# ChaoqinRobotics/LINS---LiDAR-inertial-SLAM

Hardware: AMD Instinct MI355X
Metric: ESKF iterations/sec (16x1800 VLP-16, ~2k feat) (higher is better)
Workload: dtype f64 state / f32 points

## Files before the change

### lins---lidar-inertial-slam_amd/csrc/debug_kernels.hip

```cpp
#include <hip/hip_runtime.h>

#include "ieskf_device.h"
#include "ieskf_rowsum.h"
#include "icp_wave.h"
#include "lins_launch.h"

namespace lins {

__global__ void debug_math_kernel(int op, int n, int n_in, int n_out, const double* __restrict__ in, double* __restrict__ out) {
  const int i = blockIdx.x * blockDim.x + threadIdx.x;
  if (i >= n) return;
  const double* a = in + (size_t)i * n_in;
  double* o = out + (size_t)i * n_out;
  if (op == 0) {
    const V3 v = quat2axis(Q4{a[0], a[1], a[2], a[3]});
    o[0] = v.x, o[1] = v.y, o[2] = v.z;
  } else if (op == 1) {
    const Q4 q = axis2quat(V3{a[0], a[1], a[2]});
    o[0] = q.w, o[1] = q.x, o[2] = q.y, o[3] = q.z;
  } else if (op == 2) {
    const M3 m = rinvleft(V3{a[0], a[1], a[2]});
    for (int k = 0; k < 9; ++k) o[k] = m.m[k];
  } else if (op == 3) {
    double s[19];
    for (int k = 0; k < 19; ++k) s[k] = a[k];
    box_plus_inplace(s, a + 19);
    for (int k = 0; k < 19; ++k) o[k] = s[k];
  } else if (op == 4) {
    IterConst ic;
    for (int k = 0; k < 19; ++k) ic.lin[k] = a[19 + k];
    make_iter_const(a, ic);
    for (int k = 0; k < 18; ++k) o[k] = ic.d[k];
  } else if (op == 5) {
    V3 phi;
    M3 gt;
    phi_and_Gt(Q4{a[0], a[1], a[2], a[3]}, phi, gt);
    o[0] = phi.x, o[1] = phi.y, o[2] = phi.z;
    for (int k = 0; k < 9; ++k) o[3 + k] = gt.m[k];
  } else if (op == 7) {
    double m[6][7], x6[6];
    for (int r = 0; r < 6; ++r)
      for (int c = 0; c < 7; ++c) m[r][c] = a[r * 7 + c];
    reg_solve6(m, x6);
    for (int k = 0; k < 6; ++k) o[k] = x6[k];
  } else if (op == 11) {
    double m[6][7], x6[6];
    for (int r = 0; r < 6; ++r)
      for (int c = 0; c < 7; ++c) m[r][c] = a[r * 7 + c];
    gj_solve6(m, x6);
    for (int k = 0; k < 6; ++k) o[k] = x6[k];
  } else if (op == 13) {
    const Q4 q = axis2quat_fast(V3{a[0], a[1], a[2]});
    o[0] = q.w, o[1] = q.x, o[2] = q.y, o[3] = q.z;
  } else if (op == 14) {
    const V3 v = quat2axis_fast(Q4{a[0], a[1], a[2], a[3]});
    o[0] = v.x, o[1] = v.y, o[2] = v.z;
  } else if (op == 15) {
    V3 phi;
    M3 gt;
    phi_and_Gt_general(Q4{a[0], a[1], a[2], a[3]}, phi, gt);
    o[0] = phi.x, o[1] = phi.y, o[2] = phi.z;
    for (int k = 0; k < 9; ++k) o[3 + k] = gt.m[k];
  } else if (op == 6) {
    DevParams prm{};
    prm.inv_period = (double)(1.f / (float)a[23]);
    const V3 phi = quat2axis(Q4{a[6], a[7], a[8], a[9]});
    float x, y, z;
    transform_to_start(prm, phi, V3{a[0], a[1], a[2]}, make_float4((float)a[19], (float)a[20], (float)a[21], (float)a[22]), x, y, z);
    o[0] = x, o[1] = y, o[2] = z;
  }
}

__global__ __launch_bounds__(256) void debug_cycles_kernel(int op, const double* __restrict__ in, double* __restrict__ out) {
  const int tid = threadIdx.x;
  DevParams prm{};
  prm.inv_period = 10.0, prm.icp_freq = 1, prm.lidar_scale = 1.0;
  V3 phi{in[0], in[1], in[2]}, t{in[3], in[4], in[5]};
  float4 q = make_float4((float)in[6] + tid * 0.01f, (float)in[7], (float)in[8], 3.05f);
  float acc = 0.f;
  double dacc = 0.0;
  const long long t0 = clock64();
#pragma unroll 1
  for (int r = 0; r < 64; ++r) {
    if (op == 100) {
      float x, y, z;
      transform_to_start(prm, phi, t, q, x, y, z);
      q.x = x * 0.999f + acc * 1e-9f, acc += y + z;
    } else if (op == 101) {
      QueryOut o;
      o.accepted = 0;
      o.c[0] = o.c[1] = o.c[2] = o.c[3] = 0.f;
      surf_row(prm, 1, q.x, q.y, q.z, make_float4(1.f + acc, 2.f, 3.f, 0.f), make_float4(1.5f, 2.2f, 3.f, 0.f), make_float4(1.f, 2.6f, 3.1f, 0.f), o);
      acc += o.c[0] * 1e-3f + o.c[3];
    } else if (op == 102) {
      double row[7] = {dacc + 1.0, 2.0, 3.0, 4.0, 5.0, 6.0, 7.0 + tid};
      dacc += wave_reduce_rows(row, tid & 63) * 1e-9;
    } else if (op == 103) {
      if ((tid & 63) == 0) {
        double a[6][7], x6[6];
        for (int i = 0; i < 6; ++i)
          for (int j = 0; j < 7; ++j) a[i][j] = (i == j ? 10.0 : 0.1 * (i + j)) + dacc;
        reg_solve6(a, x6);
        dacc += x6[0] * 1e-9;
      }
    } else if (op == 105) {
      const int l = tid & 63, i = l / 7, j = l % 7;
      double x6[6];
      wave_solve6(l < 42 ? (i == j ? 10.0 : 0.1 * (i + j)) + dacc : 0.0, l, x6);
      dacc += x6[0] * 1e-9;
    } else if (op == 106) {
      const int l = tid & 63, i = l / 7, j = l % 7;
      double x6[6];
      wave_gj_solve6(l < 42 ? (i == j ? 10.0 : 0.1 * (i + j)) + dacc : 0.0, l, x6);
      dacc += x6[0] * 1e-9;
    } else if (op == 107) {
      V3 p2;
      M3 gt;
      phi_and_Gt_general(Q4{1.0 - dacc, 0.01, 0.02, 0.03 + dacc}, p2, gt);
      dacc += (p2.x + gt.m[1]) * 1e-9;
    } else if (op == 108) {
      const Q4 r = axis2quat(V3{0.001 + dacc, 0.002, 0.003});
      dacc += (r.x + r.w) * 1e-9;
    } else if (op == 109) {
      const Q4 r = axis2quat_fast(V3{0.001 + dacc, 0.002, 0.003});
      dacc += (r.x + r.w) * 1e-9;
    } else if (op == 110) {
      const V3 r = quat2axis(Q4{1.0 - dacc, 0.001, 0.002, 0.003});
      dacc += r.x * 1e-9;
    } else if (op == 111) {
      const V3 r = quat2axis_fast(Q4{1.0 - dacc, 0.001, 0.002, 0.003});
      dacc += r.x * 1e-9;
    } else if (op == 104) {
      V3 p2;
      M3 gt;
      phi_and_Gt(Q4{1.0 - dacc, 0.01, 0.02, 0.03 + dacc}, p2, gt);
      dacc += (p2.x + gt.m[1]) * 1e-9;
    }
  }
  const long long t1 = clock64();
  if (tid == 0) out[blockIdx.x * 2] = (double)(t1 - t0) / 64.0, out[blockIdx.x * 2 + 1] = (double)acc + dacc;
}

__global__ void debug_wave_solve_kernel(int n, int gj, const double* __restrict__ in, double* __restrict__ out) {
  const int item = blockIdx.x, l = threadIdx.x;
  double x6[6];
  if (gj)
    wave_gj_solve6(l < 42 ? in[(size_t)item * 42 + l] : 0.0, l, x6);
  else
    wave_solve6(l < 42 ? in[(size_t)item * 42 + l] : 0.0, l, x6);
  if (l < 6) out[(size_t)item * 6 + l] = x6[l];
}
__device__ __forceinline__ double reduce_rows_ref(const double (&row)[7], int lane) {
  constexpr int A[28] = {0, 0, 0, 0, 0, 0, 1, 1, 1, 1, 1, 2, 2, 2, 2, 3, 3, 3, 4, 4, 5, 0, 1, 2, 3, 4, 5, 6};
  constexpr int B[28] = {0, 1, 2, 3, 4, 5, 1, 2, 3, 4, 5, 2, 3, 4, 5, 3, 4, 5, 4, 5, 5, 6, 6, 6, 6, 6, 6, 6};
  double v[28];
  for (int k = 0; k < 28; ++k) v[k] = row[A[k]] * row[B[k]];
  int cnt = 14;
  for (int m = 32; m >= 2; m >>= 1) {
    const bool up = (lane & m) != 0;
    if (m == 8) v[7] = 0.0;
    for (int i = 0; i < cnt; ++i) {
      const double lo = v[i], hi = v[i + cnt];
      v[i] = (up ? hi : lo) + shfl_xor_f64(up ? lo : hi, m);
    }
    cnt = m == 16 ? 4 : cnt / 2;
  }
  return v[0] + shfl_xor_f64(v[0], 1);
}
__global__ void debug_reduce_rows_kernel(int op, const double* __restrict__ in, double* __restrict__ out) {
  const int item = blockIdx.x, l = threadIdx.x;
  double row[7];
  for (int k = 0; k < 7; ++k) row[k] = in[((size_t)item * 64 + l) * 7 + k];
  const double acc = op == 9 ? wave_reduce_rows(row, l) : reduce_rows_ref(row, l);
  const int idx = reduce_sum_index(l);
  if (idx >= 0) out[(size_t)item * 28 + idx] = acc;
}
void launch_debug_reduce_rows(hipStream_t stream, int op, int n, const double* in, double* out) {
  hipLaunchKernelGGL(debug_reduce_rows_kernel, dim3(n), dim3(64), 0, stream, op, in, out);
}

__global__ void debug_icp_gn_kernel(int wave_version, const double* __restrict__ in, double* __restrict__ out) {
  __shared__ double ws[kIcpWorkspace + 48];
  const int item = blockIdx.x, l = threadIdx.x;
  const double* a = in + (size_t)item * 43;
  double* JTJ = ws + kIcpWorkspace;
  if (l < 42) JTJ[l] = a[l];
  __syncthreads();
  const int iter = (int)a[42];
  if (wave_version) {
    double x[6];
    wave_icp_gn_solve(JTJ, JTJ + 36, iter, l, x, ws);
    if (l == 0)
      for (int k = 0; k < 6; ++k) out[(size_t)item * 6 + k] = x[k];
  } else if (l == 0) {
    double* x = JTJ + 42;
    icp_gn_solve(JTJ, JTJ + 36, iter, x, ws);
    for (int k = 0; k < 6; ++k) out[(size_t)item * 6 + k] = x[k];
  }
}
void launch_debug_icp_gn(hipStream_t stream, int n, int wave_version, const double* in, double* out) {
  hipLaunchKernelGGL(debug_icp_gn_kernel, dim3(n), dim3(64), 0, stream, wave_version, in, out);
}

void launch_debug_wave_solve(hipStream_t stream, int n, int gj, const double* in, double* out) {
  hipLaunchKernelGGL(debug_wave_solve_kernel, dim3(n), dim3(64), 0, stream, n, gj, in, out);
}

void launch_debug_cycles(hipStream_t stream, int op, int blocks, const double* in, double* out) {
  hipLaunchKernelGGL(debug_cycles_kernel, dim3(blocks), dim3(256), 0, stream, op, in, out);
}

void launch_debug_math(hipStream_t stream, int op, int n, int n_in, int n_out, const double* in, double* out) {
  hipLaunchKernelGGL(debug_math_kernel, dim3((n + 63) / 64), dim3(64), 0, stream, op, n, n_in, n_out, in, out);
}

}
```

### lins---lidar-inertial-slam_amd/csrc/ieskf_rowsum.h

```cpp
#pragma once

#include <hip/hip_runtime.h>

#include "ieskf_device.h"
#include "lins_solve6.h"

namespace lins {

__device__ __forceinline__ void reg_solve6(double (&a)[6][7], double (&x)[6]) {
#pragma unroll
  for (int k = 0; k < 6; ++k) {
    int p = k;
    double best = fabs(a[k][k]);
#pragma unroll
    for (int i = k + 1; i < 6; ++i) {
      double v = fabs(a[i][k]);
      if (v > best) best = v, p = i;
    }
#pragma unroll
    for (int i = k + 1; i < 6; ++i) {
      const bool sw = (p == i);
#pragma unroll
      for (int j = k; j < 7; ++j) {
        double u = a[k][j], w = a[i][j];
        a[k][j] = sw ? w : u;
        a[i][j] = sw ? u : w;
      }
    }
    const double inv = 1.0 / a[k][k];
#pragma unroll
    for (int i = k + 1; i < 6; ++i) {
      const double f = a[i][k] * inv;
#pragma unroll
      for (int j = k + 1; j < 7; ++j) a[i][j] -= f * a[k][j];
    }
  }
#pragma unroll
  for (int i = 5; i >= 0; --i) {
    double sacc = a[i][6];
#pragma unroll
    for (int k = i + 1; k < 6; ++k) sacc -= a[i][k] * x[k];
    x[i] = sacc / a[i][i];
  }
}

__device__ __forceinline__ double shfl_f64(double v, int src) {
  const int lo = __shfl(__double2loint(v), src), hi = __shfl(__double2hiint(v), src);
  return __hiloint2double(hi, lo);
}
__device__ __forceinline__ double readlane_f64(double v, int src) {
  const int lo = __builtin_amdgcn_readlane(__double2loint(v), src), hi = __builtin_amdgcn_readlane(__double2hiint(v), src);
  return __hiloint2double(hi, lo);
}
__device__ __forceinline__ void wave_solve6(double a, int lane, double (&x)[6]) {
  const int i = lane < 42 ? lane / 7 : 7, j = lane < 42 ? lane % 7 : 0;
#pragma unroll
  for (int k = 0; k < 6; ++k) {
    int p = k;
    double best = fabs(readlane_f64(a, k * 7 + k));
#pragma unroll
    for (int r = k + 1; r < 6; ++r) {
      const double v = fabs(readlane_f64(a, r * 7 + k));
      if (v > best) best = v, p = r;
    }
    if (p != k) {
      const int src = i == k ? p * 7 + j : (i == p ? k * 7 + j : lane);
      a = shfl_f64(a, src);
    }
    const double inv = 1.0 / readlane_f64(a, k * 7 + k);
    const double aik = shfl_f64(a, (i < 6 ? i : 0) * 7 + k), akj = shfl_f64(a, k * 7 + j);
    const double f = aik * inv;
    if (i > k && i < 6 && j > k) a -= f * akj;
  }
#pragma unroll
  for (int r = 5; r >= 0; --r) {
    double sacc = readlane_f64(a, r * 7 + 6);
#pragma unroll
    for (int k = r + 1; k < 6; ++k) sacc -= readlane_f64(a, r * 7 + k) * x[k];
    x[r] = sacc / readlane_f64(a, r * 7 + r);
  }
}

__device__ __forceinline__ void wave_gj_solve6(double a, int lane, double (&x)[6]) {
  const int i = lane < 42 ? lane / 7 : 7, j = lane < 42 ? lane % 7 : 0;
#pragma unroll
  for (int k = 0; k < 6; ++k) {
    int p = k;
    unsigned best = (unsigned)__builtin_amdgcn_readlane(__double2hiint(a), k * 7 + k) & 0x7FFFFFFFu;
#pragma unroll
    for (int r = k + 1; r < 6; ++r) {
      const unsigned h = (unsigned)__builtin_amdgcn_readlane(__double2hiint(a), r * 7 + k) & 0x7FFFFFFFu;
      if (h > best) best = h, p = r;
    }
    if (p != k) {
      const int src = i == k ? p * 7 + j : (i == p ? k * 7 + j : lane);
      a = shfl_f64(a, src);
    }
    const double inv = 1.0 / readlane_f64(a, k * 7 + k);
    const double aik = shfl_f64(a, (i < 6 ? i : 0) * 7 + k), akj = shfl_f64(a, k * 7 + j);
    const double nkj = akj * inv;
    if (i < 6 && j > k) a = i == k ? nkj : a - aik * nkj;
  }
#pragma unroll
  for (int r = 0; r < 6; ++r) x[r] = readlane_f64(a, r * 7 + 6);
}

__device__ __forceinline__ double wave_gj_solve6x3(double a, int lane) {
  const int i = lane < 54 ? lane / 9 : 7, j = lane < 54 ? lane % 9 : 0;
#pragma unroll
  for (int k = 0; k < 6; ++k) {
    int p = k;
    unsigned best = (unsigned)__builtin_amdgcn_readlane(__double2hiint(a), k * 9 + k) & 0x7FFFFFFFu;
#pragma unroll
    for (int r = k + 1; r < 6; ++r) {
      const unsigned h = (unsigned)__builtin_amdgcn_readlane(__double2hiint(a), r * 9 + k) & 0x7FFFFFFFu;
      if (h > best) best = h, p = r;
    }
    if (p != k) {
      const int src = i == k ? p * 9 + j : (i == p ? k * 9 + j : lane);
      a = shfl_f64(a, src);
    }
    const double inv = 1.0 / readlane_f64(a, k * 9 + k);
    const double aik = shfl_f64(a, (i < 6 ? i : 0) * 9 + k), akj = shfl_f64(a, k * 9 + j);
    const double nkj = akj * inv;
    if (i < 6 && j > k) a = i == k ? nkj : a - aik * nkj;
  }
  return a;
}

__device__ __forceinline__ void phi_and_Gt_general(const Q4& q, V3& phi, M3& Gt) {
  const double mag = sqrt(q.x * q.x + q.y * q.y + q.z * q.z);
  phi = V3{q.x, q.y, q.z};
  Gt = M3{{1, 0, 0, 0, 1, 0, 0, 0, 1}};
  if (!(mag >= 1e-10)) return;
  const double ang = wrap_pi(2.0 * atan2(mag, q.w));
  const V3 u = V3{q.x, q.y, q.z} / mag;
  phi = ang * u;
  const double theta = norm(phi);
  if (theta < 1e-10) return;
  const double h = theta / 2.0;
  const double n = sqrt(q.w * q.w + mag * mag);
  const double s = h * ((fabs(q.w) / n) / (mag / n));
  const V3 a = V3{-phi.x, -phi.y, -phi.z} / theta;
  const M3 k = skew(a);
  const double av[3] = {a.x, a.y, a.z};
#pragma unroll
  for (int i = 0; i < 3; ++i)
#pragma unroll
    for (int jj = 0; jj < 3; ++jj)
      Gt.m[jj * 3 + i] = (s * (i == jj ? 1.0 : 0.0) + (1.0 - s) * av[i] * av[jj]) - h * k.m[i * 3 + jj];
}
__device__ __forceinline__ void phi_and_Gt(const Q4& q, V3& phi, M3& Gt) {
  if (!phi_and_gt_small(q, phi, Gt)) phi_and_Gt_general(q, phi, Gt);
}

__device__ __forceinline__ void make_iter_const_tail(const double* filt, IterConst& ic) {
  const Q4 q{ic.lin[6], ic.lin[7], ic.lin[8], ic.lin[9]};
  ic.Rt = mtrans(qmat(q));
  phi_and_Gt(q, ic.phi, ic.Gt);
  const Q4 qf{filt[6], filt[7], filt[8], filt[9]};
  const V3 da = quat2axis_fast(qmul(qinverse(q), qf));
  for (int k = 0; k < 3; ++k) {
    ic.d[0 + k] = filt[0 + k] - ic.lin[0 + k];
    ic.d[3 + k] = filt[3 + k] - ic.lin[3 + k];
    ic.d[9 + k] = filt[10 + k] - ic.lin[10 + k];
    ic.d[12 + k] = filt[13 + k] - ic.lin[13 + k];
    ic.d[15 + k] = filt[16 + k] - ic.lin[16 + k];
  }
  ic.d[6] = da.x, ic.d[7] = da.y, ic.d[8] = da.z;
}

__device__ __forceinline__ double shfl_xor_f64(double v, int mask) {
  const int lo = __shfl_xor(__double2loint(v), mask), hi = __shfl_xor(__double2hiint(v), mask);
  return __hiloint2double(hi, lo);
}
template <int MASK>
__device__ __forceinline__ int xor_lane_i32(int v, int lane) {
  if constexpr (MASK == 1) {
    return __builtin_amdgcn_mov_dpp(v, 0xB1, 0xF, 0xF, true);
  } else if constexpr (MASK == 2) {
    return __builtin_amdgcn_mov_dpp(v, 0x4E, 0xF, 0xF, true);
  } else if constexpr (MASK == 4) {
    const int r = __builtin_amdgcn_update_dpp(v, v, 0x104, 0xF, 0x5, false);
    return __builtin_amdgcn_update_dpp(r, v, 0x114, 0xF, 0xA, false);
  } else if constexpr (MASK == 8) {
    return __builtin_amdgcn_mov_dpp(v, 0x128, 0xF, 0xF, true);
  } else if constexpr (MASK == 16) {
    const auto r = __builtin_amdgcn_permlane16_swap((unsigned)v, (unsigned)v, false, false);
    return (int)((lane & 16) ? r[0] : r[1]);
  } else {
    static_assert(MASK == 32, "power of two below the wave size");
    const auto r = __builtin_amdgcn_permlane32_swap((unsigned)v, (unsigned)v, false, false);
    return (int)((lane & 32) ? r[0] : r[1]);
  }
}
template <int MASK>
__device__ __forceinline__ double xor_lane_f64(double v, int lane) {
  return __hiloint2double(xor_lane_i32<MASK>(__double2hiint(v), lane), xor_lane_i32<MASK>(__double2loint(v), lane));
}
template <int MASK>
__device__ __forceinline__ double swap_halves_add(double lo, double hi) {
  static_assert(MASK == 32 || MASK == 16, "the levels that have a lane-swap instruction");
  const unsigned ll = (unsigned)__double2loint(lo), lh = (unsigned)__double2hiint(lo);
  const unsigned hl = (unsigned)__double2loint(hi), hh = (unsigned)__double2hiint(hi);
  if constexpr (MASK == 32) {
    const auto w = __builtin_amdgcn_permlane32_swap(ll, hl, false, false), u = __builtin_amdgcn_permlane32_swap(lh, hh, false, false);
    return __hiloint2double((int)u[0], (int)w[0]) + __hiloint2double((int)u[1], (int)w[1]);
  } else {
    const auto w = __builtin_amdgcn_permlane16_swap(ll, hl, false, false), u = __builtin_amdgcn_permlane16_swap(lh, hh, false, false);
    return __hiloint2double((int)u[0], (int)w[0]) + __hiloint2double((int)u[1], (int)w[1]);
  }
}
__device__ __forceinline__ int reduce_sum_index(int lane) {
  const int local = ((lane >> 3) & 1) * 4 + ((lane >> 2) & 1) * 2 + ((lane >> 1) & 1);
  return (local < 7 && !(lane & 1)) ? ((lane >> 5) & 1) * 14 + ((lane >> 4) & 1) * 7 + local : -1;
}
__device__ __forceinline__ double wave_reduce_rows(const double (&row)[7], int lane) {
  constexpr int A[28] = {0, 0, 0, 0, 0, 0, 1, 1, 1, 1, 1, 2, 2, 2, 2, 3, 3, 3, 4, 4, 5, 0, 1, 2, 3, 4, 5, 6};
  constexpr int B[28] = {0, 1, 2, 3, 4, 5, 1, 2, 3, 4, 5, 2, 3, 4, 5, 3, 4, 5, 4, 5, 5, 6, 6, 6, 6, 6, 6, 6};
  double v[28];
#pragma unroll
  for (int k = 0; k < 28; ++k) v[k] = row[A[k]] * row[B[k]];
#pragma unroll
  for (int i = 0; i < 14; ++i) v[i] = swap_halves_add<32>(v[i], v[i + 14]);
#pragma unroll
  for (int i = 0; i < 7; ++i) v[i] = swap_halves_add<16>(v[i], v[i + 7]);
  v[7] = 0.0;
  {
    const bool up = (lane & 8) != 0;
#pragma unroll
    for (int i = 0; i < 4; ++i) {
      const double lo = v[i], hi = v[i + 4];
      v[i] = (up ? hi : lo) + xor_lane_f64<8>(up ? lo : hi, lane);
    }
  }
  {
    const bool up = (lane & 4) != 0;
#pragma unroll
    for (int i = 0; i < 2; ++i) {
      const double lo = v[i], hi = v[i + 2];
      v[i] = (up ? hi : lo) + xor_lane_f64<4>(up ? lo : hi, lane);
    }
  }
  {
    const bool up = (lane & 2) != 0;
    const double lo = v[0], hi = v[1];
    v[0] = (up ? hi : lo) + xor_lane_f64<2>(up ? lo : hi, lane);
  }
  return v[0] + xor_lane_f64<1>(v[0], lane);
}

}
```

### lins---lidar-inertial-slam_amd/csrc/lins_capi_debug.hip

```cpp
#include <vector>

#include "lins_ctx.h"
#include "lm_math.h"
#include "loop_icp.h"

using namespace lins;

extern "C" {

int lins_debug_math(lins_ctx* ctx, int op, int n, const double* in, int n_in, double* out, int n_out) {
  if (ctx && in && out && op >= 100 && op <= 111 && n >= 1 && n_in >= 9 && n_out == 2) {
    HIP_TRY(ctx, hipSetDevice(ctx->device));
    double *d_in = nullptr, *d_out = nullptr;
    HIP_TRY(ctx, hipMalloc((void**)&d_in, 9 * 8));
    HIP_TRY(ctx, hipMalloc((void**)&d_out, (size_t)n * 2 * 8));
    HIP_TRY(ctx, hipMemcpy(d_in, in, 9 * 8, hipMemcpyHostToDevice));
    launch_debug_cycles(ctx->stream, op, n, d_in, d_out);
    HIP_TRY(ctx, hipStreamSynchronize(ctx->stream));
    HIP_TRY(ctx, hipMemcpy(out, d_out, (size_t)n * 2 * 8, hipMemcpyDeviceToHost));
    (void)hipFree(d_in), (void)hipFree(d_out);
    return LINS_OK;
  }
  static const int kIn[20] = {4, 3, 3, 37, 38, 4, 24, 42, 42, 448, 448, 42, 42, 3, 4, 4, 43, 43, 72, 72};
  static const int kOut[20] = {3, 4, 9, 19, 18, 12, 3, 6, 6, 28, 28, 6, 6, 4, 3, 12, 6, 6, 44, 44};
  if (!ctx || !in || !out || op < 0 || op > 19 || n < 0 || n_in != kIn[op] || n_out != kOut[op]) return LINS_E_ARG;
  if (n == 0) return LINS_OK;
  HIP_TRY(ctx, hipSetDevice(ctx->device));
  double *d_in = nullptr, *d_out = nullptr;
  LmCarry* d_lm = nullptr;
  HIP_TRY(ctx, hipMalloc((void**)&d_in, (size_t)n * n_in * 8));
  hipError_t e = hipMalloc((void**)&d_out, (size_t)n * n_out * 8);
  if (e == hipSuccess) e = hipMemcpyAsync(d_in, in, (size_t)n * n_in * 8, hipMemcpyHostToDevice, ctx->stream);
  if (e == hipSuccess) {
    if (op == 9 || op == 10)
      launch_debug_reduce_rows(ctx->stream, op, n, d_in, d_out);
    else if (op == 8 || op == 12)
      launch_debug_wave_solve(ctx->stream, n, op == 12, d_in, d_out);
    else if (op == 16 || op == 17)
      launch_debug_icp_gn(ctx->stream, n, op == 17, d_in, d_out);
    else if (op == 18 || op == 19) {
      e = hipMalloc(&d_lm, (size_t)n * sizeof(LmCarry));
      if (e == hipSuccess) launch_debug_lm_step(ctx->stream, n, op == 19, d_in, d_out, d_lm);
    }
    else
      launch_debug_math(ctx->stream, op, n, n_in, n_out, d_in, d_out);
    e = hipGetLastError();
  }
  if (e == hipSuccess) e = hipMemcpyAsync(out, d_out, (size_t)n * n_out * 8, hipMemcpyDeviceToHost, ctx->stream);
  if (e == hipSuccess) e = hipStreamSynchronize(ctx->stream);
  (void)hipFree(d_in), (void)hipFree(d_out), (void)hipFree(d_lm);
  if (e != hipSuccess) return ctx_fail_hip(ctx, e, "lins_debug_math");
  return LINS_OK;
}

int lins_debug_scratch(lins_ctx* ctx, int which, int write, size_t offset_bytes, size_t bytes, void* host) {
  if (!ctx || !host || (which != 0 && which != 1)) return LINS_E_ARG;
  char* const base = which == 0 ? reinterpret_cast<char*>(ctx->d_relay_lane) : reinterpret_cast<char*>(ctx->d_walk_cache);
  const size_t cap = which == 0 ? (size_t)ctx->max_batch * kRelayLaneInts * sizeof(int) : ctx->slot_cap * 32;
  if (!base || offset_bytes > cap || bytes > cap - offset_bytes) return LINS_E_ARG;
  HIP_TRY(ctx, hipSetDevice(ctx->device));
  if (int rc = pipe_join(ctx)) return rc;
  if (write)
    HIP_TRY(ctx, hipMemcpyAsync(base + offset_bytes, host, bytes, hipMemcpyHostToDevice, ctx->stream));
  else
    HIP_TRY(ctx, hipMemcpyAsync(host, base + offset_bytes, bytes, hipMemcpyDeviceToHost, ctx->stream));
  HIP_TRY(ctx, hipStreamSynchronize(ctx->stream));
  return LINS_OK;
}


int lins_debug_phase_profile(lins_ctx* ctx, int enable, long long* out, int n_scans) {
  if (!ctx) return LINS_E_ARG;
  HIP_TRY(ctx, hipSetDevice(ctx->device));
  if (int rcs = split_join(ctx)) return rcs;
  if (enable && !ctx->d_prof) {
    HIP_TRY(ctx, hipMalloc((void**)&ctx->d_prof, (size_t)ctx->max_batch * 80 * sizeof(long long)));
    HIP_TRY(ctx, hipMemset(ctx->d_prof, 0, (size_t)ctx->max_batch * 80 * sizeof(long long)));
  }
  if (out && ctx->d_prof) {
    if (n_scans > ctx->max_batch) return LINS_E_CAPACITY;
    HIP_TRY(ctx, hipStreamSynchronize(ctx->stream));
    HIP_TRY(ctx, hipMemcpy(out, ctx->d_prof, (size_t)n_scans * 16 * sizeof(long long), hipMemcpyDeviceToHost));
  }
  if (!enable && ctx->d_prof) {
    (void)hipFree(ctx->d_prof);
    ctx->d_prof = nullptr;
  }
  return LINS_OK;
}

int lins_debug_queue_trace(lins_ctx* ctx, long long* out, int n_wg) {
  if (!ctx || !out || n_wg < 0) return LINS_E_ARG;
  if (!ctx->d_queue || n_wg > 15 * ctx->max_batch) return LINS_E_STATE;
  HIP_TRY(ctx, hipSetDevice(ctx->device));
  HIP_TRY(ctx, hipStreamSynchronize(ctx->stream));
  HIP_TRY(ctx, hipMemcpy(out, ctx->d_queue + lds_mr_queue_flags_offset() + (size_t)ctx->max_batch, (size_t)n_wg * 32, hipMemcpyDeviceToHost));
  return LINS_OK;
}

int lins_debug_wave_phases(lins_ctx* ctx, int* out, int n_scans) {
  if (!ctx || !out) return LINS_E_ARG;
  if (!ctx->d_prof || n_scans != ctx->n_uploaded) return LINS_E_STATE;
  HIP_TRY(ctx, hipSetDevice(ctx->device));
  HIP_TRY(ctx, hipStreamSynchronize(ctx->stream));
  HIP_TRY(ctx, hipMemcpy(out, ctx->d_prof + (size_t)n_scans * 16, (size_t)n_scans * 64 * sizeof(int), hipMemcpyDeviceToHost));
  return LINS_OK;
}

int lins_debug_wave_counts(lins_ctx* ctx, int* out, int n_scans) {
  if (!ctx || !out) return LINS_E_ARG;
  if (!ctx->d_prof || n_scans != ctx->n_uploaded) return LINS_E_STATE;
  HIP_TRY(ctx, hipSetDevice(ctx->device));
  HIP_TRY(ctx, hipStreamSynchronize(ctx->stream));
  HIP_TRY(ctx, hipMemcpy(out, ctx->d_prof + (size_t)n_scans * 48, (size_t)n_scans * 64 * sizeof(int), hipMemcpyDeviceToHost));
  return LINS_OK;
}

int lins_debug_query_slots(lins_ctx* ctx, int* out, int n_slots) {
  if (!ctx || !out || n_slots < 0 || (size_t)n_slots > ctx->slot_cap) return LINS_E_ARG;
  HIP_TRY(ctx, hipSetDevice(ctx->device));
  HIP_TRY(ctx, hipStreamSynchronize(ctx->stream));
  HIP_TRY(ctx, hipMemcpy(out, ctx->d_idx, (size_t)n_slots * sizeof(int4), hipMemcpyDeviceToHost));
  return LINS_OK;
}

int lins_debug_stream_copy(lins_ctx* ctx, uint64_t bytes, int reps, double* gbs) {
  if (!ctx || !gbs || reps < 1) return LINS_E_ARG;
  const size_t cap = ctx->arena_cap * sizeof(float4);
  if (bytes > cap) bytes = cap;
  const size_t n4 = bytes / sizeof(float4);
  if (!n4) return LINS_E_ARG;
  HIP_TRY(ctx, hipSetDevice(ctx->device));
  float best = 1e30f;
  for (int r = 0; r < reps + 1; ++r) {
    HIP_TRY(ctx, hipEventRecord(ctx->ev0, ctx->stream));
    launch_stream_copy(ctx->stream, ctx->d_arena, ctx->d_binned, n4);
    HIP_TRY(ctx, hipGetLastError());
    HIP_TRY(ctx, hipEventRecord(ctx->ev2, ctx->stream));
    HIP_TRY(ctx, hipEventSynchronize(ctx->ev2));
    float ms = 0;
    HIP_TRY(ctx, hipEventElapsedTime(&ms, ctx->ev0, ctx->ev2));
    if (r && ms < best) best = ms;
  }
  *gbs = 2.0 * (double)(n4 * sizeof(float4)) / ((double)best * 1e-3) / 1e9;
  return LINS_OK;
}

int lins_debug_pull_copy(lins_ctx* ctx, uint64_t bytes, int reps, int mode, double* gbs) {
  if (!ctx || !gbs || reps < 1) return LINS_E_ARG;
  const size_t cap = ctx->arena_cap * sizeof(float4);
  if (bytes > cap) bytes = cap;
  const size_t n4 = bytes / sizeof(float4);
  if (!n4) return LINS_E_ARG;
  HIP_TRY(ctx, hipSetDevice(ctx->device));
  if (int rc = pipe_join(ctx)) return rc;
  float4* mapped = nullptr;
  HIP_TRY(ctx, hipHostGetDevicePointer((void**)&mapped, ctx->h_arena, 0));
  float best = 1e30f;
  for (int r = 0; r < reps + 1; ++r) {
    HIP_TRY(ctx, hipEventRecord(ctx->ev0, ctx->stream));
    if (mode == 0)
      HIP_TRY(ctx, hipMemcpyAsync(ctx->d_binned, ctx->h_arena, n4 * sizeof(float4), hipMemcpyHostToDevice, ctx->stream));
    else
      launch_stream_copy(ctx->stream, mapped, ctx->d_binned, n4);
    HIP_TRY(ctx, hipGetLastError());
    HIP_TRY(ctx, hipEventRecord(ctx->ev2, ctx->stream));
    HIP_TRY(ctx, hipEventSynchronize(ctx->ev2));
    float ms = 0;
    HIP_TRY(ctx, hipEventElapsedTime(&ms, ctx->ev0, ctx->ev2));
    if (r && ms < best) best = ms;
  }
  *gbs = (double)(n4 * sizeof(float4)) / ((double)best * 1e-3) / 1e9;
  return LINS_OK;
}

int lins_debug_loop_icp_rounds(lins_ctx* ctx, int rounds) { return loop_icp_debug_set(ctx, 0, rounds); }
int lins_debug_loop_icp_shells(lins_ctx* ctx, int shells) { return loop_icp_debug_set(ctx, 1, shells < 0 ? loop_icp_debug_shells_default() : shells); }
int lins_debug_loop_icp_group(lins_ctx* ctx, int group) { return loop_icp_debug_set(ctx, 2, group); }
int lins_debug_loop_icp_last_far(lins_ctx* ctx, uint32_t* far_searches) {
  if (!ctx || !far_searches) return LINS_E_ARG;
  *far_searches = loop_icp_last_far(ctx);
  return LINS_OK;
}

int lins_debug_loop_icp_step(lins_ctx* ctx, int n, int blocks_per_problem, const int32_t* n_tiles, const int32_t* status, const double* partials,
                             const lins_loop_icp_params* prm, int mode, lins_loop_icp_state* states, int32_t* still_running) {
  if (!ctx || n < 1 || blocks_per_problem < 1 || !n_tiles || !status || !partials || !prm || (mode != 0 && mode != 1) || !states) return LINS_E_ARG;
  std::vector<LoopDev> probs(n, LoopDev{});
  std::vector<lins_licp::State> st(n);
  for (int k = 0; k < n; ++k) {
    if (n_tiles[k] < 0 || n_tiles[k] > blocks_per_problem) return LINS_E_ARG;
    probs[k].n_src = n_tiles[k] * kLoopQPerBlock, probs[k].status = status[k];
    for (int a = 0; a < 3; ++a) probs[k].g.cdim[a] = 1;
    lins_licp::state_from_public(states[k], st[k]);
  }
  HIP_TRY(ctx, hipSetDevice(ctx->device));
  const size_t np = (size_t)n * blocks_per_problem * lins_licp::kSums;
  LoopDev* d_probs = nullptr;
  lins_licp::State* d_states = nullptr;
  double* d_partials = nullptr;
  int* d_running = nullptr;
  int running = 0;
  hipError_t e = hipMalloc((void**)&d_probs, (size_t)n * sizeof(LoopDev));
  if (e == hipSuccess) e = hipMalloc((void**)&d_states, (size_t)n * sizeof(lins_licp::State));
  if (e == hipSuccess) e = hipMalloc((void**)&d_partials, np * sizeof(double));
  if (e == hipSuccess) e = hipMalloc((void**)&d_running, sizeof(int));
  if (e == hipSuccess) e = hipMemcpyAsync(d_probs, probs.data(), (size_t)n * sizeof(LoopDev), hipMemcpyHostToDevice, ctx->stream);
  if (e == hipSuccess) e = hipMemcpyAsync(d_states, st.data(), (size_t)n * sizeof(lins_licp::State), hipMemcpyHostToDevice, ctx->stream);
  if (e == hipSuccess) e = hipMemcpyAsync(d_partials, partials, np * sizeof(double), hipMemcpyHostToDevice, ctx->stream);
  if (e == hipSuccess) e = hipMemsetAsync(d_running, 0, sizeof(int), ctx->stream);
  if (e == hipSuccess) {
    launch_loop_step(ctx->stream, n, blocks_per_problem, mode, *prm, d_probs, d_states, d_partials, d_running);
    e = hipGetLastError();
  }
  if (e == hipSuccess) e = hipMemcpyAsync(st.data(), d_states, (size_t)n * sizeof(lins_licp::State), hipMemcpyDeviceToHost, ctx->stream);
  if (e == hipSuccess) e = hipMemcpyAsync(&running, d_running, sizeof(int), hipMemcpyDeviceToHost, ctx->stream);
  if (e == hipSuccess) e = hipStreamSynchronize(ctx->stream);
  (void)hipFree(d_probs), (void)hipFree(d_states), (void)hipFree(d_partials), (void)hipFree(d_running);
  if (e != hipSuccess) return ctx_fail_hip(ctx, e, "lins_debug_loop_icp_step");
  for (int k = 0; k < n; ++k) lins_licp::state_to_public(st[k], states[k]);
  if (still_running) *still_running = running;
  return LINS_OK;
}

int lins_debug_cov_update(lins_ctx* ctx, int path, int n, const double* P, const double* sums, double r2, const int32_t* diverged, double* out) {
  if (!ctx || path < 0 || path > 3 || n < 1 || !P || !sums || !diverged || !out) return LINS_E_ARG;
  HIP_TRY(ctx, hipSetDevice(ctx->device));
  std::vector<OutRec> recs(n, OutRec{});
  for (int k = 0; k < n; ++k) recs[k].diverged = diverged[k] != 0;
  double *d_P = nullptr, *d_sums = nullptr, *d_out = nullptr;
  int* d_div = nullptr;
  OutRec* d_recs = nullptr;
  hipError_t e = hipMalloc((void**)&d_P, (size_t)n * 324 * 8);
  if (e == hipSuccess) e = hipMalloc((void**)&d_sums, (size_t)n * 21 * 8);
  if (e == hipSuccess) e = hipMalloc((void**)&d_out, (size_t)n * 324 * 8);
  if (e == hipSuccess) e = hipMalloc((void**)&d_div, (size_t)n * sizeof(int));
  if (e == hipSuccess) e = hipMalloc((void**)&d_recs, (size_t)n * sizeof(OutRec));
  if (e == hipSuccess) e = hipMemcpyAsync(d_P, P, (size_t)n * 324 * 8, hipMemcpyHostToDevice, ctx->stream);
  if (e == hipSuccess) e = hipMemcpyAsync(d_sums, sums, (size_t)n * 21 * 8, hipMemcpyHostToDevice, ctx->stream);
  if (e == hipSuccess) e = hipMemcpyAsync(d_div, diverged, (size_t)n * sizeof(int), hipMemcpyHostToDevice, ctx->stream);
  if (e == hipSuccess) e = hipMemcpyAsync(d_recs, recs.data(), (size_t)n * sizeof(OutRec), hipMemcpyHostToDevice, ctx->stream);
  if (e == hipSuccess) e = hipMemsetAsync(d_out, 0xFF, (size_t)n * 324 * 8, ctx->stream);
  if (e == hipSuccess) {
    if (path == 3) {
      DevParams prm{};
      prm.r2 = r2;
      launch_joseph(ctx->stream, n, prm, d_P, d_sums, d_recs, d_out);
    } else if (path == 2) {
      launch_debug_cov_lds_mr(ctx->stream, n, r2, d_P, d_sums, d_div, d_out);
    } else {
      launch_debug_cov_lds(ctx->stream, n, path == 0 ? 3 : 1, r2, d_P, d_sums, d_div, d_out);
    }
    e = hipGetLastError();
  }
  if (e == hipSuccess) e = hipMemcpyAsync(out, d_out, (size_t)n * 324 * 8, hipMemcpyDeviceToHost, ctx->stream);
  if (e == hipSuccess) e = hipStreamSynchronize(ctx->stream);
  (void)hipFree(d_P), (void)hipFree(d_sums), (void)hipFree(d_out), (void)hipFree(d_div), (void)hipFree(d_recs);
  if (e != hipSuccess) return ctx_fail_hip(ctx, e, "lins_debug_cov_update");
  return LINS_OK;
}

}
```

Baseline: 22.12 million.

## Replace row-swap pivoting in wave Gauss-Jordan solves with index-tracked pivoting

The wave-level 6x7 and 6x9 Gauss-Jordan solvers no longer physically swap rows through a shuffle when pivoting. They keep a row_of permutation, find candidate pivots with a ballot over the lanes still open, and compute the reciprocal speculatively alongside the bpermute loads. This removes the extra cross-lane shuffle and the serial chain of readlanes on the pivot path, at the cost of more complex index logic and a final permuted gather. Debug ops are added to test the 6x3 variant.

After: 22.19 million, median of 6. About the same (+0.3%).

```diff
diff --git a/lins---lidar-inertial-slam_amd/csrc/debug_kernels.hip b/lins---lidar-inertial-slam_amd/csrc/debug_kernels.hip
--- a/lins---lidar-inertial-slam_amd/csrc/debug_kernels.hip
+++ b/lins---lidar-inertial-slam_amd/csrc/debug_kernels.hip
@@ -113,6 +113,10 @@
       double x6[6];
       wave_gj_solve6(l < 42 ? (i == j ? 10.0 : 0.1 * (i + j)) + dacc : 0.0, l, x6);
       dacc += x6[0] * 1e-9;
+    } else if (op == 112) {
+      const int l = tid & 63, i = l / 9, j = l % 9;
+      const double r = wave_gj_solve6x3(l < 54 ? (i == j ? 10.0 : (j < 6 ? 0.1 * (i + j) : (i == j - 6 ? 1.0 : 0.0))) + dacc : 0.0, l);
+      dacc += readlane_f64(r, 6) * 1e-9;
     } else if (op == 107) {
       V3 p2;
       M3 gt;
@@ -143,6 +147,11 @@
 
 __global__ void debug_wave_solve_kernel(int n, int gj, const double* __restrict__ in, double* __restrict__ out) {
   const int item = blockIdx.x, l = threadIdx.x;
+  if (gj == 2) {
+    const double v = wave_gj_solve6x3(l < 54 ? in[(size_t)item * 54 + l] : 0.0, l);
+    if (l < 54 && l % 9 >= 6) out[(size_t)item * 18 + (l / 9) * 3 + (l % 9 - 6)] = v;
+    return;
+  }
   double x6[6];
   if (gj)
     wave_gj_solve6(l < 42 ? in[(size_t)item * 42 + l] : 0.0, l, x6);
diff --git a/lins---lidar-inertial-slam_amd/csrc/ieskf_rowsum.h b/lins---lidar-inertial-slam_amd/csrc/ieskf_rowsum.h
--- a/lins---lidar-inertial-slam_amd/csrc/ieskf_rowsum.h
+++ b/lins---lidar-inertial-slam_amd/csrc/ieskf_rowsum.h
@@ -81,51 +81,66 @@
   }
 }
 
+__device__ __forceinline__ double bpermute_f64(double v, int byte_addr) {
+  const int lo = __builtin_amdgcn_ds_bpermute(byte_addr, __double2loint(v)), hi = __builtin_amdgcn_ds_bpermute(byte_addr, __double2hiint(v));
+  return __hiloint2double(hi, lo);
+}
+template <int W>
+__device__ __forceinline__ double wave_gj_columns(double a, int lane, int (&row_of)[6]) {
+  const int i = lane < 6 * W ? lane / W : 7, j = lane < 6 * W ? lane % W : 0;
+  const int own = (i < 6 ? i : 0) * W, col = j * 4;
+#pragma unroll
+  for (int r = 0; r < 6; ++r) row_of[r] = r * W;
+  unsigned long long open = 0;
+#pragma unroll
+  for (int r = 0; r < 6; ++r) open |= 1ull << (r * W);
+#pragma unroll
+  for (int k = 0; k < 6; ++k) {
+    const int first = row_of[k];
+    const double aik = bpermute_f64(a, own * 4 + k * 4);
+    double akj = bpermute_f64(a, first * 4 + col);
+    __builtin_amdgcn_sched_barrier(0);
+    double rcp = 1.0 / a;
+    const unsigned h = (unsigned)__double2hiint(a) & 0x7FFFFFFFu;
+    const unsigned h_first = k < 5 ? (unsigned)__builtin_amdgcn_readlane((int)h, first + k) : 0u;
+    const unsigned long long above = k < 5 ? __ballot(h > h_first) & open : 0ull;
+    asm volatile("" : "+v"(rcp));
+    int pr = first;
+    if (above) {
+      unsigned best = h_first;
+#pragma unroll
+      for (int r = k + 1; r < 6; ++r) {
+        const int cand = row_of[r];
+        const unsigned hc = (unsigned)__builtin_amdgcn_readlane((int)h, cand + k);
+        if (hc > best) best = hc, pr = cand;
+      }
+#pragma unroll
+      for (int r = k + 1; r < 6; ++r) row_of[r] = row_of[r] == pr ? first : row_of[r];
+      row_of[k] = pr;
+      akj = bpermute_f64(a, pr * 4 + col);
+    }
+    open = (open & ~(1ull << (pr + k))) << 1;
+    const double inv = readlane_f64(rcp, pr + k);
+    const double nkj = akj * inv;
+    if (j > k) a = own == pr ? nkj : a - aik * nkj;
+  }
+  return a;
+}
 __device__ __forceinline__ void wave_gj_solve6(double a, int lane, double (&x)[6]) {
-  const int i = lane < 42 ? lane / 7 : 7, j = lane < 42 ? lane % 7 : 0;
-#pragma unroll
-  for (int k = 0; k < 6; ++k) {
-    int p = k;
-    unsigned best = (unsigned)__builtin_amdgcn_readlane(__double2hiint(a), k * 7 + k) & 0x7FFFFFFFu;
-#pragma unroll
-    for (int r = k + 1; r < 6; ++r) {
-      const unsigned h = (unsigned)__builtin_amdgcn_readlane(__double2hiint(a), r * 7 + k) & 0x7FFFFFFFu;
-      if (h > best) best = h, p = r;
-    }
-    if (p != k) {
-      const int src = i == k ? p * 7 + j : (i == p ? k * 7 + j : lane);
-      a = shfl_f64(a, src);
-    }
-    const double inv = 1.0 / readlane_f64(a, k * 7 + k);
-    const double aik = shfl_f64(a, (i < 6 ? i : 0) * 7 + k), akj = shfl_f64(a, k * 7 + j);
-    const double nkj = akj * inv;
-    if (i < 6 && j > k) a = i == k ? nkj : a - aik * nkj;
-  }
-#pragma unroll
-  for (int r = 0; r < 6; ++r) x[r] = readlane_f64(a, r * 7 + 6);
+  int row_of[6];
+  a = wave_gj_columns<7>(a, lane, row_of);
+#pragma unroll
+  for (int r = 0; r < 6; ++r) x[r] = readlane_f64(a, row_of[r] + 6);
 }
 
 __device__ __forceinline__ double wave_gj_solve6x3(double a, int lane) {
-  const int i = lane < 54 ? lane / 9 : 7, j = lane < 54 ? lane % 9 : 0;
-#pragma unroll
-  for (int k = 0; k < 6; ++k) {
-    int p = k;
-    unsigned best = (unsigned)__builtin_amdgcn_readlane(__double2hiint(a), k * 9 + k) & 0x7FFFFFFFu;
-#pragma unroll
-    for (int r = k + 1; r < 6; ++r) {
-      const unsigned h = (unsigned)__builtin_amdgcn_readlane(__double2hiint(a), r * 9 + k) & 0x7FFFFFFFu;
-      if (h > best) best = h, p = r;
-    }
-    if (p != k) {
-      const int src = i == k ? p * 9 + j : (i == p ? k * 9 + j : lane);
-      a = shfl_f64(a, src);
-    }
-    const double inv = 1.0 / readlane_f64(a, k * 9 + k);
-    const double aik = shfl_f64(a, (i < 6 ? i : 0) * 9 + k), akj = shfl_f64(a, k * 9 + j);
-    const double nkj = akj * inv;
-    if (i < 6 && j > k) a = i == k ? nkj : a - aik * nkj;
-  }
-  return a;
+  int row_of[6];
+  a = wave_gj_columns<9>(a, lane, row_of);
+  const int i = lane < 54 ? lane / 9 : 0, j = lane < 54 ? lane % 9 : 0;
+  int src = row_of[0];
+#pragma unroll
+  for (int r = 1; r < 6; ++r) src = i == r ? row_of[r] : src;
+  return bpermute_f64(a, (src + j) * 4);
 }
 
 __device__ __forceinline__ void phi_and_Gt_general(const Q4& q, V3& phi, M3& Gt) {
diff --git a/lins---lidar-inertial-slam_amd/csrc/lins_capi_debug.hip b/lins---lidar-inertial-slam_amd/csrc/lins_capi_debug.hip
--- a/lins---lidar-inertial-slam_amd/csrc/lins_capi_debug.hip
+++ b/lins---lidar-inertial-slam_amd/csrc/lins_capi_debug.hip
@@ -9,7 +9,7 @@
 extern "C" {
 
 int lins_debug_math(lins_ctx* ctx, int op, int n, const double* in, int n_in, double* out, int n_out) {
-  if (ctx && in && out && op >= 100 && op <= 111 && n >= 1 && n_in >= 9 && n_out == 2) {
+  if (ctx && in && out && op >= 100 && op <= 112 && n >= 1 && n_in >= 9 && n_out == 2) {
     HIP_TRY(ctx, hipSetDevice(ctx->device));
     double *d_in = nullptr, *d_out = nullptr;
     HIP_TRY(ctx, hipMalloc((void**)&d_in, 9 * 8));
@@ -21,9 +21,9 @@
     (void)hipFree(d_in), (void)hipFree(d_out);
     return LINS_OK;
   }
-  static const int kIn[20] = {4, 3, 3, 37, 38, 4, 24, 42, 42, 448, 448, 42, 42, 3, 4, 4, 43, 43, 72, 72};
-  static const int kOut[20] = {3, 4, 9, 19, 18, 12, 3, 6, 6, 28, 28, 6, 6, 4, 3, 12, 6, 6, 44, 44};
-  if (!ctx || !in || !out || op < 0 || op > 19 || n < 0 || n_in != kIn[op] || n_out != kOut[op]) return LINS_E_ARG;
+  static const int kIn[21] = {4, 3, 3, 37, 38, 4, 24, 42, 42, 448, 448, 42, 42, 3, 4, 4, 43, 43, 72, 72, 54};
+  static const int kOut[21] = {3, 4, 9, 19, 18, 12, 3, 6, 6, 28, 28, 6, 6, 4, 3, 12, 6, 6, 44, 44, 18};
+  if (!ctx || !in || !out || op < 0 || op > 20 || n < 0 || n_in != kIn[op] || n_out != kOut[op]) return LINS_E_ARG;
   if (n == 0) return LINS_OK;
   HIP_TRY(ctx, hipSetDevice(ctx->device));
   double *d_in = nullptr, *d_out = nullptr;
@@ -34,8 +34,8 @@
   if (e == hipSuccess) {
     if (op == 9 || op == 10)
       launch_debug_reduce_rows(ctx->stream, op, n, d_in, d_out);
-    else if (op == 8 || op == 12)
-      launch_debug_wave_solve(ctx->stream, n, op == 12, d_in, d_out);
+    else if (op == 8 || op == 12 || op == 20)
+      launch_debug_wave_solve(ctx->stream, n, op == 20 ? 2 : op == 12, d_in, d_out);
     else if (op == 16 || op == 17)
       launch_debug_icp_gn(ctx->stream, n, op == 17, d_in, d_out);
     else if (op == 18 || op == 19) {
```
